# halide/Halide

Measured on AMD Instinct MI355X. Metric: megapixels/sec local_laplacian 8-level fp32 4K, higher is better.
Workload: dtype f32; 1 GPU; apps/local_laplacian J=8 levels=8 alpha=1/7 beta=1, u16 RGB planar 3840x2160; distinct_frames_per_gpu=8, lut_cached=True, streams_per_gpu=4, frame_scheduling=4 frame-queue streams, boundary=C ABI local_laplacian(halide_buffer_t*,int32,float,float,halide_buffer_t*), rccl_ranks=1, parallelism=frames sharded over 1 GPU(s), no data-path collective

## Files before the change

### halide_amd/csrc/local_laplacian.hip

```cpp
#include "hlmi_device_math.h"
#include "hlmi_internal.h"

#include <atomic>
#include <mutex>
#include <optional>
#include <stdlib.h>
#include <string.h>
#include <type_traits>

using namespace hlmi;

namespace {

constexpr int J = 8;
constexpr int MAX_K = 32;
constexpr int STRIP = 126;
constexpr int KCH = 8;
constexpr int D0_THREADS = 256;

struct Level {
    int lox, loy;
    int w, h;
    int ws;
    size_t ps;
// ... 2007 lines not shown
        stage1(y + 2, f0, s0, g0);
        __builtin_amdgcn_sched_barrier(0);
        stage2(y + 1, s1, g1);
        __builtin_amdgcn_sched_barrier(0);
    }
    LL_PROBE_T(pt3);
    LL_PROBE_ADD(8, pt1 - pt0); LL_PROBE_ADD(9, pt2 - pt1); LL_PROBE_ADD(10, 1);
    LL_PROBE_ADD(11, pt3 - pt2); LL_PROBE_ADD(12, pt3 - pt0);
}

struct Up0HArgs {
    Up0Args u;
    const float *outl0;
    int l0_ws;
    int fuse2;
    const float *g3, *out3;
    int lox3, loy3, ws3;
    size_t ps3;
};
constexpr int U0H_PF = 4;
constexpr int U0H_T2 = 68;
template<bool NT, bool EM1, int CH = 2>
__global__ __launch_bounds__(256) void ll_up0h(Up0HArgs ph, Geometry gm) {
    const Up0Args &p = ph.u;
    LL_RESIDENCY(1);
    extern __shared__ float s_out1[];
    int bx, by;
    {
        const int b = (int)blockIdx.y * (int)gridDim.x + (int)blockIdx.x, nb8 = (int)(gridDim.x * gridDim.y) >> 3;
        const int lb = b < (nb8 << 3) ? (b & 7) * nb8 + (b >> 3) : b;
        by = lb / (int)gridDim.x, bx = lb - by * (int)gridDim.x;
    }
    const int X0 = p.ox0 + bx * 256;
    const int Yw0 = p.oy0 + by * (2 * p.RU);
    const int Yw1 = min(Yw0 + 2 * p.RU, p.oy0 + p.oh) - 1;
    const int cx0 = (X0 >> 1) - 1, cy0 = dev::fdiv2(Yw0 - 1);
    const int th = dev::fdiv2(Yw1 + 1) - cy0 + 1;
    float *const s_out2 = s_out1 + U0_TS * (p.RU + 2);
    const int cx1 = min(cx0 + U0_TW - 1, p.rx1_1);
    const int c2x0 = dev::fdiv2(cx0 - 1), c2y0 = dev::fdiv2(cy0 - 1);
    struct Taps32 {
        uint32_t b, a;
    };
    auto mul24 = [](uint32_t a, uint32_t b) { return (uint32_t)__umul24(a, b); };
    auto tap_bytes = [&](uint32_t row0, int y0, int lox, int ws, int X, int Y) {
        Taps32 t;
        t.b = (row0 + mul24((uint32_t)(dev::fdiv2(Y - 1) - y0), (uint32_t)ws) + (uint32_t)(dev::fdiv2(X - 1) - lox)) << 2;
        t.a = t.b + ((uint32_t)ws << 2);
        return t;
    };
    auto taps_at = [](const float *base, uint32_t plane_bytes, const Taps32 &t) {
        const F2U lo = ld_su<F2U>(base, plane_bytes + t.b), hi = ld_su<F2U>(base, plane_bytes + t.a);
        UpTaps r;
        r.bb = lo.x, r.ba = lo.y, r.ab = hi.x, r.aa = hi.y;
        return r;
    };
    const uint32_t ps1b = (uint32_t)p.ps1 * 4u, ps2b = (uint32_t)p.ps2 * 4u, ps3b = (uint32_t)ph.ps3 * 4u;
    if (ph.fuse2) {
        const int n2x = dev::fdiv2(cx1 + 1) - c2x0 + 1, n2y = dev::fdiv2(cy0 + th) - c2y0 + 1, n2 = n2x * n2y;
        const uint32_t m2 = (4194304u + (uint32_t)n2x - 1u) / (uint32_t)n2x;
        const int c3y0 = dev::fdiv2(c2y0 - 1);
        const uint32_t row2 = (uint32_t)((c2y0 - p.loy2) * p.ws2), row3 = (uint32_t)((c3y0 - ph.loy3) * ph.ws3);
        for (int e0 = threadIdx.x; e0 < n2; e0 += 256 * CH) {
            int X2[CH], Y2[CH];
            uint32_t ti[CH];
            bool ok[CH];
            uint32_t ob[CH];
            Taps32 t3[CH];
            float inG[CH], lf[CH], ga[CH], gb[CH];
            UpTaps o3[CH], t0[CH], t1[CH];
#pragma unroll
            for (int i = 0; i < CH; i++) {
                const int e = e0 + 256 * i;
                const uint32_t ec = (uint32_t)min(e, n2 - 1), ty = mul24(ec, m2) >> 22, tx = ec - mul24(ty, (uint32_t)n2x);
                ok[i] = e < n2, ti[i] = mul24(ty, U0H_T2) + tx;
                X2[i] = c2x0 + (int)tx, Y2[i] = c2y0 + (int)ty;
                ob[i] = (row2 + mul24(ty, (uint32_t)p.ws2) + (uint32_t)(X2[i] - p.lox2)) << 2;
                inG[i] = ld_su<float>(p.g2, (uint32_t)gm.K * ps2b + ob[i]);
                t3[i] = tap_bytes(row3, c3y0, ph.lox3, ph.ws3, X2[i], Y2[i]);
                o3[i] = taps_at(ph.out3, 0u, t3[i]);
            }
            __builtin_amdgcn_sched_barrier(0);
#pragma unroll
            for (int i = 0; i < CH; i++) {
                const float level = inG[i] * gm.Km1;
                const int li = dev::clampi((int)level, 0, gm.K - 2);
                lf[i] = level - (float)li;
                ga[i] = ld_su<float>(p.g2, (uint32_t)li * ps2b + ob[i]), gb[i] = ld_su<float>(p.g2, (uint32_t)(li + 1) * ps2b + ob[i]);
                t0[i] = taps_at(ph.g3, (uint32_t)li * ps3b, t3[i]);
                t1[i] = taps_at(ph.g3, (uint32_t)(li + 1) * ps3b, t3[i]);
            }
            __builtin_amdgcn_sched_barrier(0);
#pragma unroll
            for (int i = 0; i < CH; i++) {
                const float l0 = ga[i] - up_from(t0[i], X2[i], Y2[i]), l1 = gb[i] - up_from(t1[i], X2[i], Y2[i]);
                const float outL = dev::mad2(1.0f - lf[i], l0, lf[i], l1);
                if (ok[i]) s_out2[ti[i]] = up_from(o3[i], X2[i], Y2[i]) + outL;
            }
        }
        __syncthreads();
    }
    {
        const int n1 = U0_TW * th;
        constexpr uint32_t M1 = (4194304u + U0_TW - 1) / U0_TW;
        const uint32_t row1 = (uint32_t)((cy0 - p.loy1) * p.ws1), row2 = (uint32_t)((c2y0 - p.loy2) * p.ws2);
        if constexpr (EM1) {
            for (int e0 = threadIdx.x; e0 < n1; e0 += 256 * CH) {
                int cx[CH], cy[CH];
                uint32_t ti[CH];
                bool ok[CH];
                float outL[CH];
#pragma unroll
                for (int i = 0; i < CH; i++) {
                    const int e = e0 + 256 * i;
                    const uint32_t ec = (uint32_t)min(e, n1 - 1), ty = mul24(ec, M1) >> 22, tx = ec - mul24(ty, U0_TW);
                    ok[i] = e < n1 && cx0 + (int)tx <= p.rx1_1, ti[i] = mul24(ty, U0_TS) + tx;
                    cx[i] = min(cx0 + (int)tx, p.rx1_1), cy[i] = cy0 + (int)ty;
                    outL[i] = ld_su<float>(p.g1, (row1 + mul24(ty, (uint32_t)p.ws1) + (uint32_t)(cx[i] - p.lox1)) << 2);
                }
#pragma unroll
                for (int i = 0; i < CH; i++) {
                    const float *q = s_out2 + mul24((uint32_t)(dev::fdiv2(cy[i] - 1) - c2y0), U0H_T2) + (uint32_t)(dev::fdiv2(cx[i] - 1) - c2x0);
                    UpTaps t;
                    t.bb = q[0], t.ba = q[1], t.ab = q[U0H_T2], t.aa = q[U0H_T2 + 1];
                    if (ok[i]) s_out1[ti[i]] = up_from(t, cx[i], cy[i]) + outL[i];
                }
            }
        } else {
            for (int e0 = threadIdx.x; e0 < n1; e0 += 256 * CH) {
                int cx[CH], cy[CH];
                uint32_t ti[CH];
                bool ok[CH];
                Taps32 t2[CH];
                float inG[CH], lf[CH], ga[CH], gb[CH];
                UpTaps o2[CH], t0[CH], t1[CH];
#pragma unroll
                for (int i = 0; i < CH; i++) {
                    const int e = e0 + 256 * i;
                    const uint32_t ec = (uint32_t)min(e, n1 - 1), ty = mul24(ec, M1) >> 22, tx = ec - mul24(ty, U0_TW);
                    ok[i] = e < n1 && cx0 + (int)tx <= p.rx1_1, ti[i] = mul24(ty, U0_TS) + tx;
                    cx[i] = min(cx0 + (int)tx, p.rx1_1), cy[i] = cy0 + (int)ty;
                    const uint32_t ob = (row1 + mul24(ty, (uint32_t)p.ws1) + (uint32_t)(cx[i] - p.lox1)) << 2;
                    inG[i] = ld_su<float>(p.g1, (uint32_t)gm.K * ps1b + ob), ga[i] = ld_su<float>(p.g1, ob), gb[i] = ld_su<float>(p.g1, ps1b + ob);
                    t2[i] = tap_bytes(row2, c2y0, p.lox2, p.ws2, cx[i], cy[i]);
                    if (!ph.fuse2) o2[i] = taps_at(p.out2, 0u, t2[i]);
                }
                __builtin_amdgcn_sched_barrier(0);
#pragma unroll
                for (int i = 0; i < CH; i++) {
                    const float level = inG[i] * gm.Km1;
                    const int li = dev::clampi((int)level, 0, gm.K - 2);
                    lf[i] = level - (float)li;
                    t0[i] = taps_at(p.g2, (uint32_t)li * ps2b, t2[i]);
                    t1[i] = taps_at(p.g2, (uint32_t)(li + 1) * ps2b, t2[i]);
                }
                __builtin_amdgcn_sched_barrier(0);
#pragma unroll
                for (int i = 0; i < CH; i++) {
                    const float l0 = ga[i] - up_from(t0[i], cx[i], cy[i]), l1 = gb[i] - up_from(t1[i], cx[i], cy[i]);
                    const float outL = dev::mad2(1.0f - lf[i], l0, lf[i], l1);
                    float up2;
                    if (ph.fuse2) {
                        const float *q = s_out2 + mul24((uint32_t)(dev::fdiv2(cy[i] - 1) - c2y0), U0H_T2) + (uint32_t)(dev::fdiv2(cx[i] - 1) - c2x0);
                        UpTaps t;
                        t.bb = q[0], t.ba = q[1], t.ab = q[U0H_T2], t.aa = q[U0H_T2 + 1];
                        up2 = up_from(t, cx[i], cy[i]);
                    } else {
                        up2 = up_from(o2[i], cx[i], cy[i]);
                    }
                    if (ok[i]) s_out1[ti[i]] = up2 + outL;
                }
            }
        }
    }
    __syncthreads();
    const int wave = __builtin_amdgcn_readfirstlane(threadIdx.x >> 6), lane = threadIdx.x & 63;
    const int x = bx * 256 + (wave & 1) * 128 + 2 * lane;
    const int y0 = by * (2 * p.RU) + (wave >> 1) * p.RU;
    if (y0 >= p.oh || x >= p.ow) return;
    const int y1 = min(y0 + p.RU, p.oh);
    const int X = p.ox0 + x;
    uint32_t inb = (uint32_t)(X - gm.ix0) * 2u, outb = (uint32_t)x * 2u, l0b = (uint32_t)(X - gm.ix0) * 4u;
    auto hl0 = [](float rm, float r0) {
        return dev::CANON_FMA ? __builtin_fmaf(r0, 0.75f, rm * 0.25f) : __builtin_fmaf(rm, 0.25f, r0 * 0.75f);
    };
    auto hl1 = [](float r0, float rp) { return __builtin_fmaf(rp, 0.25f, r0 * 0.75f); };
    auto vl = [](float uq, float ut, float wq, float wt) {
        return dev::CANON_FMA ? __builtin_fmaf(uq, wq, ut * wt) : __builtin_fmaf(uq, 0.25f, ut * 0.75f);
    };
    struct Frame {
        ushort2 c0, c1, c2;
        float2 l0;
    };
    auto fresh = [](uint32_t &v) {
        asm volatile("" : "+v"(v));
        return v;
    };
    auto load_frame = [&](int y, Frame &f) {
        const int yc = min(y, y1 - 1);
        const uint16_t *irow = p.in + (long)(p.oy0 + yc - gm.iy0) * p.in_sy;
        const uint32_t ib = fresh(inb);
        f.c0 = ld_frame2<NT>(irow + p.gco[0], ib), f.c1 = ld_frame2<NT>(irow + p.gco[1], ib), f.c2 = ld_frame2<NT>(irow + p.gco[2], ib);
        {
            const f2 *const lp = reinterpret_cast<const f2 *>(reinterpret_cast<const char *>(ph.outl0 + (size_t)yc * ph.l0_ws) + fresh(l0b));
            const f2 v = NT ? __builtin_nontemporal_load(lp) : *lp;
            f.l0 = make_float2(v.x, v.y);
        }
    };
    auto finish = [&](int y, const Frame &f) {
        const int Y = p.oy0 + min(y, y1 - 1);
        const int ya = dev::fdiv2(Y + 1), yb = dev::fdiv2(Y - 1);
        const bool yodd = dev::fmod2(Y) != 0;
        const int yq = (dev::CANON_FMA || yodd) ? ya : yb, yt = (dev::CANON_FMA || yodd) ? yb : ya;
        const float wq = yodd ? 0.25f : 0.75f, wt = yodd ? 0.75f : 0.25f;
        const float *oa = s_out1 + (yq - cy0) * U0_TS + (wave & 1) * 64 + lane;
        const float *ob = s_out1 + (yt - cy0) * U0_TS + (wave & 1) * 64 + lane;
        const float ax = oa[0], ay = oa[1], az = oa[2], bx = ob[0], by = ob[1], bz = ob[2];
        const float uo[2] = {vl(hl0(ax, ay), hl0(bx, by), wq, wt), vl(hl1(ay, az), hl1(by, bz), wq, wt)};
        const float outL[2] = {f.l0.x, f.l0.y};
        const uint16_t ch[3][2] = {{f.c0.x, f.c0.y}, {f.c1.x, f.c1.y}, {f.c2.x, f.c2.y}};
        uint16_t res[3][2];
#pragma unroll
        for (int i = 0; i < 2; i++) {
            const float gray = gray_from(ch[0][i], ch[1][i], ch[2][i]);
            const float og = (uo[i] + outL[i]) + 0.01f;
            const float gr = gray + 0.01f;
            const float n[3] = {(float)ch[0][i] * og, (float)ch[1][i] * og, (float)ch[2][i] * og};
            float q[3];
            div3_by(n, gr, q);
#pragma unroll
            for (int c = 0; c < 3; c++) res[c][i] = (uint16_t)__builtin_amdgcn_fmed3f(q[c], 0.0f, 65535.0f);
        }
        if (y < y1) {
            uint16_t *orow = p.out + (long)y * p.out_sy;
#pragma unroll
            for (int c = 0; c < 3; c++) st_frame2<NT>(reinterpret_cast<char *>(orow + (long)c * p.out_sc) + fresh(outb), res[c][0], res[c][1]);
        }
    };
    Frame f[U0H_PF];
#pragma unroll
    for (int i = 0; i < U0H_PF; i++) load_frame(y0 + i, f[i]);
    for (int y = y0; y < y1; y += U0H_PF) {
#pragma unroll
        for (int i = 0; i < U0H_PF; i++) {
            const Frame cur = f[i];
            load_frame(y + U0H_PF + i, f[i]);
            finish(y + i, cur);
        }
    }
}

const ArgTable ll_table("local_laplacian", {
    in_buf("input", T_U16, 3, {0, 1536, 0, 2560, 0, 3}),
    scalar_i32("levels").estimate(8),
    scalar_f32("alpha").estimate(1),
    scalar_f32("beta").estimate(1),
    out_buf("output", T_U16, 3, {0, 1536, 0, 2560, 0, 3}),
});

struct LlSwitches {
    std::optional<int> fuse_from, upchain_from, ru, units0, no_vec, emit, nt, fuse_up2, d01_exch, d01_pad_lds, no_lut_cache, emit1, chain_fit;
};
LlSwitches ll_switches() {
    const auto get = env_int;
    LlSwitches s;
    s.fuse_from = get("HLMI_LL_FUSE_FROM"), s.upchain_from = get("HLMI_LL_UPCHAIN_FROM");
    s.ru = get("HLMI_LL_RU"), s.units0 = get("HLMI_LL_UNITS0"), s.no_vec = get("HLMI_LL_NO_VEC");
    s.emit = get("HLMI_LL_EMIT"), s.nt = get("HLMI_LL_NT"), s.fuse_up2 = get("HLMI_LL_FUSE_UP2");
    s.d01_exch = get("HLMI_LL_D01_EXCH"), s.d01_pad_lds = get("HLMI_LL_D01_PAD_LDS"), s.no_lut_cache = get("HLMI_LL_NO_LUT_CACHE");
    s.emit1 = get("HLMI_LL_EMIT1"), s.chain_fit = get("HLMI_LL_CHAIN_FIT");
    return s;
}

int dev_clamp_ru(int ru) { return ru < 1 ? 1 : (ru > 300 ? 300 : ru); }

struct PairGeom {
    int S2;
    int Pbase;
    int nsx;
};
struct LlPlan {
    Geometry gm;
    Level lv[J];
    size_t off_g[J], off_out[J], off_l0, ws_floats;
    Up0Args u0;
    int nlut;
    int S, SU;
    int up_low;
    bool lut_cache;
    bool lut_lds;
    bool vec_frame;
    bool vec_in;
    bool b1;
    bool fast, fuse1, fuse2, emit, nt;
    bool emit1;
    bool d01;
    bool strip2;
    bool chain_fit;
    struct { PairGeom pg; bool exch; int nsy, nunits; size_t lds; } d0;
    struct { PairGeom pg; int nsy, nunits; } s2;
    int units_strip;
    size_t up0_lds;
};

struct LlBuffers {
    float *lut, *outl0;
    float *g[J], *outg[J];
};

PairGeom pair_geom(const Level &d, const Level &e, int fewer = 0) {
    PairGeom g;
    g.S2 = ((d.odd || e.odd) ? 62 : 61) - fewer;
    const int lim = e.odd ? 2 * e.lox - 1 : 2 * e.lox - 2;
    g.Pbase = min(d.lox, lim);
    const int hi1 = d.lox + d.w - 1, hi2 = e.lox + e.w - 1;
    const int x2_first = e.odd ? (g.Pbase + 1) / 2 + 0 : g.Pbase / 2 + 1;
    g.nsx = max((hi2 - x2_first + g.S2) / g.S2, (hi1 - g.Pbase + 2 * g.S2) / (2 * g.S2));
    return g;
// ... 67 lines not shown
        const int v = sw.upchain_from.value_or(S == 4 ? 3 : 0);
        return (v >= 1 && v <= J - 2) ? v : S;
    }();
    const bool partitioned = stream_cus < device_cus;
    bool vec_frame = (din % 4 == 0) && (dout % 4 == 0) && in_sy % 2 == 0 && out_sy % 2 == 0 && out_sc % 2 == 0 &&
                     ((p.ox0 - gm.ix0) % 2 == 0) && !sw.no_vec.value_or(0);
    for (int ch = 0; ch < 3; ch++) vec_frame = vec_frame && p.gco[ch] % 2 == 0 && p.cco[ch] % 2 == 0;
    pl.vec_frame = vec_frame;
    const bool vec_in = pl.vec_in = (din % 8 == 0) && in_sy % 4 == 0 && p.gco[0] % 4 == 0 && p.gco[1] % 4 == 0 && p.gco[2] % 4 == 0 &&
                                    iw % 4 == 0 && !sw.no_vec.value_or(0);
    const bool fast = pl.fast = vec_frame && same && nc == 3 && (ow & 1) == 0 && (p.ox0 & 1) == 0 &&
                                (double)(levels + 1) * (4.0 * (double)lv[1].ps) < 4.0e9;
    const bool fuse1 = pl.fuse1 = fast && SU >= 2;
    const bool d01 = pl.d01 = levels == KCH && lut_lds && vec_in;
    const bool emit = pl.emit = d01 && fast && fuse1 && lv[1].ws < (1 << 24) && sw.emit.value_or(1);
    int RU = dev_clamp_ru(sw.ru.value_or(emit ? (partitioned ? 32 : 8) : fuse1 ? (partitioned ? 32 : 16) : 8));
    pl.nt = sw.nt.value_or(partitioned ? 1 : 0) != 0;
    pl.fuse2 = emit && SU >= 3 && SU < J && sw.fuse_up2.value_or(1);
    pl.up_low = fuse1 ? (pl.fuse2 ? 3 : 2) : 1;
    constexpr bool kEmit1Default = true;
    constexpr size_t kCuLds = 160 * 1024, kLdsGranule = 1280;
    constexpr int WPB = D0_THREADS / 64;
    auto lds_alloc = [](size_t bytes) { return (bytes + kLdsGranule - 1) / kLdsGranule * kLdsGranule; };
    auto up0h_lds = [](int ru) { return sizeof(float) * ((size_t)U0_TS * (ru + 2) + (size_t)U0H_T2 * (ru / 2 + 4)); };
    const size_t d01_lds_exch = sizeof(float) * ((nlut + 1) & ~1) + sizeof(float2) * D01_STATE * (2 * WPB - 1);
    pl.emit1 = false;
    {
        const int e1 = sw.emit1.value_or(-1);
        if (pl.fuse2 && (e1 > 0 || (e1 < 0 && partitioned && kEmit1Default))) {
            const size_t d0 = lds_alloc(d01_lds_exch + d01_em1_lds_bytes());
            auto fits = [&](int ru) { return d0 + 3 * lds_alloc(up0h_lds(ru)) <= kCuLds; };
            int ru = RU;
            if (partitioned && !sw.ru) {
                ru &= ~3;
                while (ru > 8 && !fits(ru)) ru -= 4;
            }
            pl.emit1 = e1 > 0 || fits(ru);
            if (pl.emit1) RU = ru;
        }
    }
    p.RU = RU;
    pl.strip2 = d01 && S == 4;

    pl.off_l0 = ws_floats;
    if (emit) ws_floats += ((size_t)iw * (size_t)oh + 63) & ~(size_t)63;
    pl.ws_floats = ws_floats;

    if (!d01) {
        const Level &d = lv[1];
        const int target = sw.units0.value_or(8 * device_cus);
        pl.d0.nsy = max(1, min(max(target / d.nsx, (d.h + 63) / 64), max(1, d.h / 2)));
        pl.d0.nunits = d.nsx * pl.d0.nsy;
        pl.d0.lds = (lut_lds ? sizeof(float) * ((nlut + 1) & ~1) : 0) + sizeof(float2) * D0_THREADS * (KCH + 1);
    } else {
        const Level &e = lv[2];
        const PairGeom pg = pl.d0.pg = pair_geom(lv[1], e, pl.emit1 ? (e.odd ? 1 : 2) : 0);
        const int target2 = sw.units0.value_or(emit && partitioned ? 10 * stream_cus : 8 * device_cus);
        bool exch = sw.d01_exch.value_or(1) != 0;
        int nwy = 0;
        auto ceil_div = [](int x, int y) { return (x + y - 1) / y; };
        if (exch) {
            const int nwy_max = max(1, target2 / (WPB * pg.nsx));
            const int n = max(2, (ceil_div(e.h, nwy_max) + 1 + 3) / 4);
// ... 2 lines not shown
        }
        pl.d0.exch = exch;
        if (exch) {
            pl.d0.nsy = nwy;
            pl.d0.nunits = pg.nsx * nwy * WPB;
        } else {
            pl.d0.nsy = max(1, min(max(target2 / pg.nsx, (e.h + 31) / 32), e.h));
            pl.d0.nunits = pg.nsx * pl.d0.nsy;
        }
        size_t sh2 = sizeof(float) * ((nlut + 1) & ~1) + sizeof(float2) * D01_STATE * (WPB + (exch ? WPB - 1 : 0));
        if (pl.emit1) sh2 += d01_em1_lds_bytes();
        const int pad = sw.d01_pad_lds.value_or(emit && partitioned ? -1 : 0);
        constexpr size_t kHalfCuLds = 160 * 1024 / 2;
        if (pad < 0) sh2 = max(sh2, kHalfCuLds + 2048);
        else sh2 += (size_t)pad;
        pl.d0.lds = sh2;
    }
    if (pl.strip2) {
        pl.s2.pg = pair_geom(lv[3], lv[4]);
        pl.s2.nsy = (lv[4].h + S2_RPU - 1) / S2_RPU;
        pl.s2.nunits = (levels + 1) * pl.s2.pg.nsx * pl.s2.nsy;
    }
    pl.units_strip = 16 * device_cus;
    pl.up0_lds = emit   ? sizeof(float) * ((size_t)U0_TS * (RU + 2) + (size_t)U0H_T2 * (RU / 2 + 4))
                 : fast ? lut_sh + (fuse1 ? ((lut_lds && (nlut & 1)) ? 4 : 0) + sizeof(float) * U0_TS * (RU + 2) : 0)
                        : lut_sh;
    {
        const int cf = (double)(levels + 1) * (4.0 * (double)lv[1].ps) < 4.0e9 ? sw.chain_fit.value_or(-1) : 0;
        const size_t taken = lds_alloc(pl.d0.lds) + 3 * lds_alloc(pl.up0_lds);
        const size_t need = max(S < J - 1 ? lds_alloc(dm_lds_bytes(J - 1 - S)) : (size_t)0, SU < J - 1 ? lds_alloc(um_lds_bytes(J - 1 - SU)) : (size_t)0);
        pl.chain_fit = cf > 0 || (cf < 0 && pl.emit1 && partitioned && taken + need <= kCuLds);
    }
}

struct LlLastCall {
    LlPlan pl;
    LlBuffers b;
    hipStream_t stream;
    bool out1_pending;
    bool out2_pending;
};
thread_local LlLastCall t_dbg = {};

StripArgs strip_args(const LlPlan &pl, const LlBuffers &b, int j) {
    const Level &sl = pl.lv[j], &d = pl.lv[j + 1];
    const int cols = d.nsx * (pl.gm.K + 1);
    StripArgs a;
// ... 179 lines not shown
        HLMI_LAUNCH(uc, nm, st, ll_up<false>, dim3((ua.rw + 255) / 256, ua.rh), dim3(256), 0, ua);
    }
    return 0;
}

int ll_stage_up0(void *uc, const LlPlan &pl, const LlBuffers &b, hipStream_t st) {
    const Geometry &gm = pl.gm;
    const Level *lv = pl.lv;
    const Level &c = lv[1];
    Up0Args p = pl.u0;
    const int ow = p.ow, oh = p.oh, nc = p.nc;
    p.lut_g = b.lut, p.g1 = b.g[1], p.out1 = b.outg[1];
    p.lox1 = c.lox, p.loy1 = c.loy, p.ws1 = c.ws, p.ps1 = c.ps;
    p.g2 = b.g[2], p.out2 = b.outg[2], p.lox2 = lv[2].lox, p.loy2 = lv[2].loy, p.ws2 = lv[2].ws, p.ps2 = lv[2].ps;
    p.rx1_1 = c.rx1, p.rx0_1 = c.rx0, p.ry0_1 = c.ry0, p.ry1_1 = c.ry1;
    dim3 grid((ow + 255) / 256, (oh + 2 * p.RU - 1) / (2 * p.RU)), block(256);
    const double n1 = (double)(c.rx1 - c.rx0 + 1) * (c.ry1 - c.ry0 + 1), n2 = (double)(lv[2].rx1 - lv[2].rx0 + 1) * (lv[2].ry1 - lv[2].ry0 + 1);
    if (pl.emit) {
        timing_note_bytes(2.0 * (3 + nc) * ow * oh + 4.0 * ow * oh + 4.0 * (pl.emit1 ? 1.0 : 3.0) * n1 + 4.0 * 3.0 * n2);
        Up0HArgs ph;
        ph.u = p, ph.outl0 = b.outl0, ph.l0_ws = gm.ix1 - gm.ix0 + 1;
        ph.fuse2 = pl.fuse2 ? 1 : 0;
        ph.g3 = b.g[3], ph.out3 = b.outg[3], ph.lox3 = lv[3].lox, ph.loy3 = lv[3].loy, ph.ws3 = lv[3].ws, ph.ps3 = lv[3].ps;
        return with_flags([&](auto NT, auto E1) -> int {
            HLMI_LAUNCH(uc, "ll_up0", st, (ll_up0h<NT.value, E1.value>), grid, block, pl.up0_lds, ph, gm);
            return 0;
        }, pl.nt, pl.emit1);
    }
    timing_note_bytes(2.0 * (3 + nc) * ow * oh + 4.0 * 3.0 * n1 + (pl.fuse1 ? 4.0 * 3.0 * n2 : 0.0));
    if (pl.fast) {
        return with_flags([&](auto L, auto B, auto F) -> int {
            HLMI_LAUNCH(uc, "ll_up0", st, (ll_up0f<L.value, B.value, F.value>), grid, block, pl.up0_lds, p, gm);
            return 0;
        }, pl.lut_lds, pl.b1, pl.fuse1);
    }
    return with_flags([&](auto V, auto L) -> int {
        HLMI_LAUNCH(uc, "ll_up0", st, (ll_up0<V.value, L.value>), grid, block, pl.up0_lds, p, gm);
        return 0;
    }, pl.vec_frame, pl.lut_lds);
}

}

extern "C" int local_laplacian(halide_buffer_t *input, int32_t levels, float alpha, float beta, halide_buffer_t *output) {
    void *uc = nullptr;
    const LlSwitches sw = ll_switches();
// ... 169 lines not shown
```

Measured before the change: 125,400 Mpx/s.

## Stream level-1 rows per wave in up0h instead of staging a full LDS tile

Adds an ll_up0r variant of the fused level-0 upsample kernel. It computes level-1 coarse rows on the fly, one row per wave, using DPP lane shifts plus a small per-wave edge buffer for horizontal neighbours, instead of first materialising the whole level-1 tile in LDS. This shrinks per-block LDS, which lets the planner use a taller RU (64) while still fitting three blocks per CU. The cost is a more complex kernel with wave-level synchronisation, and horizontal-edge values get recomputed. The variant is enabled by default on partitioned emit1 plans.

```diff
diff --git a/halide_amd/csrc/local_laplacian.hip b/halide_amd/csrc/local_laplacian.hip
--- a/halide_amd/csrc/local_laplacian.hip
+++ b/halide_amd/csrc/local_laplacian.hip
@@ -2053,232 +2053,14 @@
 constexpr int U0H_T2 = 68;
 template<bool NT, bool EM1, int CH = 2>
 __global__ __launch_bounds__(256) void ll_up0h(Up0HArgs ph, Geometry gm) {
-    const Up0Args &p = ph.u;
-    LL_RESIDENCY(1);
-    extern __shared__ float s_out1[];
-    int bx, by;
-    {
-        const int b = (int)blockIdx.y * (int)gridDim.x + (int)blockIdx.x, nb8 = (int)(gridDim.x * gridDim.y) >> 3;
-        const int lb = b < (nb8 << 3) ? (b & 7) * nb8 + (b >> 3) : b;
-        by = lb / (int)gridDim.x, bx = lb - by * (int)gridDim.x;
-    }
-    const int X0 = p.ox0 + bx * 256;
-    const int Yw0 = p.oy0 + by * (2 * p.RU);
-    const int Yw1 = min(Yw0 + 2 * p.RU, p.oy0 + p.oh) - 1;
-    const int cx0 = (X0 >> 1) - 1, cy0 = dev::fdiv2(Yw0 - 1);
-    const int th = dev::fdiv2(Yw1 + 1) - cy0 + 1;
-    float *const s_out2 = s_out1 + U0_TS * (p.RU + 2);
-    const int cx1 = min(cx0 + U0_TW - 1, p.rx1_1);
-    const int c2x0 = dev::fdiv2(cx0 - 1), c2y0 = dev::fdiv2(cy0 - 1);
-    struct Taps32 {
-        uint32_t b, a;
-    };
-    auto mul24 = [](uint32_t a, uint32_t b) { return (uint32_t)__umul24(a, b); };
-    auto tap_bytes = [&](uint32_t row0, int y0, int lox, int ws, int X, int Y) {
-        Taps32 t;
-        t.b = (row0 + mul24((uint32_t)(dev::fdiv2(Y - 1) - y0), (uint32_t)ws) + (uint32_t)(dev::fdiv2(X - 1) - lox)) << 2;
-        t.a = t.b + ((uint32_t)ws << 2);
-        return t;
-    };
-    auto taps_at = [](const float *base, uint32_t plane_bytes, const Taps32 &t) {
-        const F2U lo = ld_su<F2U>(base, plane_bytes + t.b), hi = ld_su<F2U>(base, plane_bytes + t.a);
-        UpTaps r;
-        r.bb = lo.x, r.ba = lo.y, r.ab = hi.x, r.aa = hi.y;
-        return r;
-    };
-    const uint32_t ps1b = (uint32_t)p.ps1 * 4u, ps2b = (uint32_t)p.ps2 * 4u, ps3b = (uint32_t)ph.ps3 * 4u;
-    if (ph.fuse2) {
-        const int n2x = dev::fdiv2(cx1 + 1) - c2x0 + 1, n2y = dev::fdiv2(cy0 + th) - c2y0 + 1, n2 = n2x * n2y;
-        const uint32_t m2 = (4194304u + (uint32_t)n2x - 1u) / (uint32_t)n2x;
-        const int c3y0 = dev::fdiv2(c2y0 - 1);
-        const uint32_t row2 = (uint32_t)((c2y0 - p.loy2) * p.ws2), row3 = (uint32_t)((c3y0 - ph.loy3) * ph.ws3);
-        for (int e0 = threadIdx.x; e0 < n2; e0 += 256 * CH) {
-            int X2[CH], Y2[CH];
-            uint32_t ti[CH];
-            bool ok[CH];
-            uint32_t ob[CH];
-            Taps32 t3[CH];
-            float inG[CH], lf[CH], ga[CH], gb[CH];
-            UpTaps o3[CH], t0[CH], t1[CH];
-#pragma unroll
-            for (int i = 0; i < CH; i++) {
-                const int e = e0 + 256 * i;
-                const uint32_t ec = (uint32_t)min(e, n2 - 1), ty = mul24(ec, m2) >> 22, tx = ec - mul24(ty, (uint32_t)n2x);
-                ok[i] = e < n2, ti[i] = mul24(ty, U0H_T2) + tx;
-                X2[i] = c2x0 + (int)tx, Y2[i] = c2y0 + (int)ty;
-                ob[i] = (row2 + mul24(ty, (uint32_t)p.ws2) + (uint32_t)(X2[i] - p.lox2)) << 2;
-                inG[i] = ld_su<float>(p.g2, (uint32_t)gm.K * ps2b + ob[i]);
-                t3[i] = tap_bytes(row3, c3y0, ph.lox3, ph.ws3, X2[i], Y2[i]);
-                o3[i] = taps_at(ph.out3, 0u, t3[i]);
-            }
-            __builtin_amdgcn_sched_barrier(0);
-#pragma unroll
-            for (int i = 0; i < CH; i++) {
-                const float level = inG[i] * gm.Km1;
-                const int li = dev::clampi((int)level, 0, gm.K - 2);
-                lf[i] = level - (float)li;
-                ga[i] = ld_su<float>(p.g2, (uint32_t)li * ps2b + ob[i]), gb[i] = ld_su<float>(p.g2, (uint32_t)(li + 1) * ps2b + ob[i]);
-                t0[i] = taps_at(ph.g3, (uint32_t)li * ps3b, t3[i]);
-                t1[i] = taps_at(ph.g3, (uint32_t)(li + 1) * ps3b, t3[i]);
-            }
-            __builtin_amdgcn_sched_barrier(0);
-#pragma unroll
-            for (int i = 0; i < CH; i++) {
-                const float l0 = ga[i] - up_from(t0[i], X2[i], Y2[i]), l1 = gb[i] - up_from(t1[i], X2[i], Y2[i]);
-                const float outL = dev::mad2(1.0f - lf[i], l0, lf[i], l1);
-                if (ok[i]) s_out2[ti[i]] = up_from(o3[i], X2[i], Y2[i]) + outL;
-            }
-        }
-        __syncthreads();
-    }
-    {
-        const int n1 = U0_TW * th;
-        constexpr uint32_t M1 = (4194304u + U0_TW - 1) / U0_TW;
-        const uint32_t row1 = (uint32_t)((cy0 - p.loy1) * p.ws1), row2 = (uint32_t)((c2y0 - p.loy2) * p.ws2);
-        if constexpr (EM1) {
-            for (int e0 = threadIdx.x; e0 < n1; e0 += 256 * CH) {
-                int cx[CH], cy[CH];
-                uint32_t ti[CH];
-                bool ok[CH];
-                float outL[CH];
-#pragma unroll
-                for (int i = 0; i < CH; i++) {
-                    const int e = e0 + 256 * i;
-                    const uint32_t ec = (uint32_t)min(e, n1 - 1), ty = mul24(ec, M1) >> 22, tx = ec - mul24(ty, U0_TW);
-                    ok[i] = e < n1 && cx0 + (int)tx <= p.rx1_1, ti[i] = mul24(ty, U0_TS) + tx;
-                    cx[i] = min(cx0 + (int)tx, p.rx1_1), cy[i] = cy0 + (int)ty;
-                    outL[i] = ld_su<float>(p.g1, (row1 + mul24(ty, (uint32_t)p.ws1) + (uint32_t)(cx[i] - p.lox1)) << 2);
-                }
-#pragma unroll
-                for (int i = 0; i < CH; i++) {
-                    const float *q = s_out2 + mul24((uint32_t)(dev::fdiv2(cy[i] - 1) - c2y0), U0H_T2) + (uint32_t)(dev::fdiv2(cx[i] - 1) - c2x0);
-                    UpTaps t;
-                    t.bb = q[0], t.ba = q[1], t.ab = q[U0H_T2], t.aa = q[U0H_T2 + 1];
-                    if (ok[i]) s_out1[ti[i]] = up_from(t, cx[i], cy[i]) + outL[i];
-                }
-            }
-        } else {
-            for (int e0 = threadIdx.x; e0 < n1; e0 += 256 * CH) {
-                int cx[CH], cy[CH];
-                uint32_t ti[CH];
-                bool ok[CH];
-                Taps32 t2[CH];
-                float inG[CH], lf[CH], ga[CH], gb[CH];
-                UpTaps o2[CH], t0[CH], t1[CH];
-#pragma unroll
-                for (int i = 0; i < CH; i++) {
-                    const int e = e0 + 256 * i;
-                    const uint32_t ec = (uint32_t)min(e, n1 - 1), ty = mul24(ec, M1) >> 22, tx = ec - mul24(ty, U0_TW);
-                    ok[i] = e < n1 && cx0 + (int)tx <= p.rx1_1, ti[i] = mul24(ty, U0_TS) + tx;
-                    cx[i] = min(cx0 + (int)tx, p.rx1_1), cy[i] = cy0 + (int)ty;
-                    const uint32_t ob = (row1 + mul24(ty, (uint32_t)p.ws1) + (uint32_t)(cx[i] - p.lox1)) << 2;
-                    inG[i] = ld_su<float>(p.g1, (uint32_t)gm.K * ps1b + ob), ga[i] = ld_su<float>(p.g1, ob), gb[i] = ld_su<float>(p.g1, ps1b + ob);
-                    t2[i] = tap_bytes(row2, c2y0, p.lox2, p.ws2, cx[i], cy[i]);
-                    if (!ph.fuse2) o2[i] = taps_at(p.out2, 0u, t2[i]);
-                }
-                __builtin_amdgcn_sched_barrier(0);
-#pragma unroll
-                for (int i = 0; i < CH; i++) {
-                    const float level = inG[i] * gm.Km1;
-                    const int li = dev::clampi((int)level, 0, gm.K - 2);
-                    lf[i] = level - (float)li;
-                    t0[i] = taps_at(p.g2, (uint32_t)li * ps2b, t2[i]);
-                    t1[i] = taps_at(p.g2, (uint32_t)(li + 1) * ps2b, t2[i]);
-                }
-                __builtin_amdgcn_sched_barrier(0);
-#pragma unroll
-                for (int i = 0; i < CH; i++) {
-                    const float l0 = ga[i] - up_from(t0[i], cx[i], cy[i]), l1 = gb[i] - up_from(t1[i], cx[i], cy[i]);
-                    const float outL = dev::mad2(1.0f - lf[i], l0, lf[i], l1);
-                    float up2;
-                    if (ph.fuse2) {
-                        const float *q = s_out2 + mul24((uint32_t)(dev::fdiv2(cy[i] - 1) - c2y0), U0H_T2) + (uint32_t)(dev::fdiv2(cx[i] - 1) - c2x0);
-                        UpTaps t;
-                        t.bb = q[0], t.ba = q[1], t.ab = q[U0H_T2], t.aa = q[U0H_T2 + 1];
-                        up2 = up_from(t, cx[i], cy[i]);
-                    } else {
-                        up2 = up_from(o2[i], cx[i], cy[i]);
-                    }
-                    if (ok[i]) s_out1[ti[i]] = up2 + outL;
-                }
-            }
-        }
-    }
-    __syncthreads();
-    const int wave = __builtin_amdgcn_readfirstlane(threadIdx.x >> 6), lane = threadIdx.x & 63;
-    const int x = bx * 256 + (wave & 1) * 128 + 2 * lane;
-    const int y0 = by * (2 * p.RU) + (wave >> 1) * p.RU;
-    if (y0 >= p.oh || x >= p.ow) return;
-    const int y1 = min(y0 + p.RU, p.oh);
-    const int X = p.ox0 + x;
-    uint32_t inb = (uint32_t)(X - gm.ix0) * 2u, outb = (uint32_t)x * 2u, l0b = (uint32_t)(X - gm.ix0) * 4u;
-    auto hl0 = [](float rm, float r0) {
-        return dev::CANON_FMA ? __builtin_fmaf(r0, 0.75f, rm * 0.25f) : __builtin_fmaf(rm, 0.25f, r0 * 0.75f);
-    };
-    auto hl1 = [](float r0, float rp) { return __builtin_fmaf(rp, 0.25f, r0 * 0.75f); };
-    auto vl = [](float uq, float ut, float wq, float wt) {
-        return dev::CANON_FMA ? __builtin_fmaf(uq, wq, ut * wt) : __builtin_fmaf(uq, 0.25f, ut * 0.75f);
-    };
-    struct Frame {
-        ushort2 c0, c1, c2;
-        float2 l0;
-    };
-    auto fresh = [](uint32_t &v) {
-        asm volatile("" : "+v"(v));
-        return v;
-    };
-    auto load_frame = [&](int y, Frame &f) {
-        const int yc = min(y, y1 - 1);
-        const uint16_t *irow = p.in + (long)(p.oy0 + yc - gm.iy0) * p.in_sy;
-        const uint32_t ib = fresh(inb);
-        f.c0 = ld_frame2<NT>(irow + p.gco[0], ib), f.c1 = ld_frame2<NT>(irow + p.gco[1], ib), f.c2 = ld_frame2<NT>(irow + p.gco[2], ib);
-        {
-            const f2 *const lp = reinterpret_cast<const f2 *>(reinterpret_cast<const char *>(ph.outl0 + (size_t)yc * ph.l0_ws) + fresh(l0b));
-            const f2 v = NT ? __builtin_nontemporal_load(lp) : *lp;
-            f.l0 = make_float2(v.x, v.y);
-        }
-    };
-    auto finish = [&](int y, const Frame &f) {
-        const int Y = p.oy0 + min(y, y1 - 1);
-        const int ya = dev::fdiv2(Y + 1), yb = dev::fdiv2(Y - 1);
-        const bool yodd = dev::fmod2(Y) != 0;
-        const int yq = (dev::CANON_FMA || yodd) ? ya : yb, yt = (dev::CANON_FMA || yodd) ? yb : ya;
-        const float wq = yodd ? 0.25f : 0.75f, wt = yodd ? 0.75f : 0.25f;
-        const float *oa = s_out1 + (yq - cy0) * U0_TS + (wave & 1) * 64 + lane;
-        const float *ob = s_out1 + (yt - cy0) * U0_TS + (wave & 1) * 64 + lane;
-        const float ax = oa[0], ay = oa[1], az = oa[2], bx = ob[0], by = ob[1], bz = ob[2];
-        const float uo[2] = {vl(hl0(ax, ay), hl0(bx, by), wq, wt), vl(hl1(ay, az), hl1(by, bz), wq, wt)};
-        const float outL[2] = {f.l0.x, f.l0.y};
-        const uint16_t ch[3][2] = {{f.c0.x, f.c0.y}, {f.c1.x, f.c1.y}, {f.c2.x, f.c2.y}};
-        uint16_t res[3][2];
-#pragma unroll
-        for (int i = 0; i < 2; i++) {
-            const float gray = gray_from(ch[0][i], ch[1][i], ch[2][i]);
-            const float og = (uo[i] + outL[i]) + 0.01f;
-            const float gr = gray + 0.01f;
-            const float n[3] = {(float)ch[0][i] * og, (float)ch[1][i] * og, (float)ch[2][i] * og};
-            float q[3];
-            div3_by(n, gr, q);
-#pragma unroll
-            for (int c = 0; c < 3; c++) res[c][i] = (uint16_t)__builtin_amdgcn_fmed3f(q[c], 0.0f, 65535.0f);
-        }
-        if (y < y1) {
-            uint16_t *orow = p.out + (long)y * p.out_sy;
-#pragma unroll
-            for (int c = 0; c < 3; c++) st_frame2<NT>(reinterpret_cast<char *>(orow + (long)c * p.out_sc) + fresh(outb), res[c][0], res[c][1]);
-        }
-    };
-    Frame f[U0H_PF];
-#pragma unroll
-    for (int i = 0; i < U0H_PF; i++) load_frame(y0 + i, f[i]);
-    for (int y = y0; y < y1; y += U0H_PF) {
-#pragma unroll
-        for (int i = 0; i < U0H_PF; i++) {
-            const Frame cur = f[i];
-            load_frame(y + U0H_PF + i, f[i]);
-            finish(y + i, cur);
-        }
-    }
+    constexpr bool ROWS1 = false;
+#include "local_laplacian_up0h_body.h"
+}
+template<bool NT>
+__global__ __launch_bounds__(256) void ll_up0r(Up0HArgs ph, Geometry gm) {
+    constexpr bool EM1 = true, ROWS1 = true;
+    constexpr int CH = 2;
+#include "local_laplacian_up0h_body.h"
 }
 
 const ArgTable ll_table("local_laplacian", {
@@ -2290,7 +2072,7 @@
 });
 
 struct LlSwitches {
-    std::optional<int> fuse_from, upchain_from, ru, units0, no_vec, emit, nt, fuse_up2, d01_exch, d01_pad_lds, no_lut_cache, emit1, chain_fit;
+    std::optional<int> fuse_from, upchain_from, ru, units0, no_vec, emit, nt, fuse_up2, d01_exch, d01_pad_lds, no_lut_cache, emit1, chain_fit, up1_rows;
 };
 LlSwitches ll_switches() {
     const auto get = env_int;
@@ -2299,7 +2081,7 @@
     s.ru = get("HLMI_LL_RU"), s.units0 = get("HLMI_LL_UNITS0"), s.no_vec = get("HLMI_LL_NO_VEC");
     s.emit = get("HLMI_LL_EMIT"), s.nt = get("HLMI_LL_NT"), s.fuse_up2 = get("HLMI_LL_FUSE_UP2");
     s.d01_exch = get("HLMI_LL_D01_EXCH"), s.d01_pad_lds = get("HLMI_LL_D01_PAD_LDS"), s.no_lut_cache = get("HLMI_LL_NO_LUT_CACHE");
-    s.emit1 = get("HLMI_LL_EMIT1"), s.chain_fit = get("HLMI_LL_CHAIN_FIT");
+    s.emit1 = get("HLMI_LL_EMIT1"), s.chain_fit = get("HLMI_LL_CHAIN_FIT"), s.up1_rows = get("HLMI_LL_UP1_ROWS");
     return s;
 }
 
@@ -2325,6 +2107,7 @@
     bool b1;
     bool fast, fuse1, fuse2, emit, nt;
     bool emit1;
+    bool up1_rows;
     bool d01;
     bool strip2;
     bool chain_fit;
@@ -2438,16 +2221,22 @@
     constexpr size_t kCuLds = 160 * 1024, kLdsGranule = 1280;
     constexpr int WPB = D0_THREADS / 64;
     auto lds_alloc = [](size_t bytes) { return (bytes + kLdsGranule - 1) / kLdsGranule * kLdsGranule; };
-    auto up0h_lds = [](int ru) { return sizeof(float) * ((size_t)U0_TS * (ru + 2) + (size_t)U0H_T2 * (ru / 2 + 4)); };
+    auto up0h_lds = [](int ru, bool rows1) {
+        return sizeof(float) * ((rows1 ? (size_t)(256 / 64) * 2 * (ru / 2 + 2) : (size_t)U0_TS * (ru + 2)) + (size_t)U0H_T2 * (ru / 2 + 4));
+    };
     const size_t d01_lds_exch = sizeof(float) * ((nlut + 1) & ~1) + sizeof(float2) * D01_STATE * (2 * WPB - 1);
+    constexpr int kRows1Ru = 64;
     pl.emit1 = false;
+    bool rows1 = false;
     {
-        const int e1 = sw.emit1.value_or(-1);
+        const int e1 = sw.emit1.value_or(-1), u1 = sw.up1_rows.value_or(-1);
         if (pl.fuse2 && (e1 > 0 || (e1 < 0 && partitioned && kEmit1Default))) {
+            rows1 = u1 > 0 || (u1 < 0 && partitioned);
             const size_t d0 = lds_alloc(d01_lds_exch + d01_em1_lds_bytes());
-            auto fits = [&](int ru) { return d0 + 3 * lds_alloc(up0h_lds(ru)) <= kCuLds; };
+            auto fits = [&](int ru) { return d0 + 3 * lds_alloc(up0h_lds(ru, rows1)) <= kCuLds; };
             int ru = RU;
             if (partitioned && !sw.ru) {
+                if (rows1) ru = kRows1Ru;
                 ru &= ~3;
                 while (ru > 8 && !fits(ru)) ru -= 4;
             }
@@ -2455,6 +2244,7 @@
             if (pl.emit1) RU = ru;
         }
     }
+    pl.up1_rows = pl.emit1 && rows1;
     p.RU = RU;
     pl.strip2 = d01 && S == 4;
 
@@ -2503,7 +2293,7 @@
         pl.s2.nunits = (levels + 1) * pl.s2.pg.nsx * pl.s2.nsy;
     }
     pl.units_strip = 16 * device_cus;
-    pl.up0_lds = emit   ? sizeof(float) * ((size_t)U0_TS * (RU + 2) + (size_t)U0H_T2 * (RU / 2 + 4))
+    pl.up0_lds = emit   ? up0h_lds(RU, pl.up1_rows)
                  : fast ? lut_sh + (fuse1 ? ((lut_lds && (nlut & 1)) ? 4 : 0) + sizeof(float) * U0_TS * (RU + 2) : 0)
                         : lut_sh;
     {
@@ -2729,6 +2519,12 @@
         ph.u = p, ph.outl0 = b.outl0, ph.l0_ws = gm.ix1 - gm.ix0 + 1;
         ph.fuse2 = pl.fuse2 ? 1 : 0;
         ph.g3 = b.g[3], ph.out3 = b.outg[3], ph.lox3 = lv[3].lox, ph.loy3 = lv[3].loy, ph.ws3 = lv[3].ws, ph.ps3 = lv[3].ps;
+        if (pl.up1_rows) {
+            return with_flags([&](auto NT) -> int {
+                HLMI_LAUNCH(uc, "ll_up0r", st, (ll_up0r<NT.value>), grid, block, pl.up0_lds, ph, gm);
+                return 0;
+            }, pl.nt);
+        }
         return with_flags([&](auto NT, auto E1) -> int {
             HLMI_LAUNCH(uc, "ll_up0", st, (ll_up0h<NT.value, E1.value>), grid, block, pl.up0_lds, ph, gm);
             return 0;
diff --git a/halide_amd/csrc/local_laplacian_up0h_body.h b/halide_amd/csrc/local_laplacian_up0h_body.h
--- /dev/null
+++ b/halide_amd/csrc/local_laplacian_up0h_body.h
@@ -0,0 +1,326 @@
+    static_assert(EM1 || !ROWS1, "ROWS1 adds the stored outLPyramid[1] plane");
+    const Up0Args &p = ph.u;
+    LL_RESIDENCY(1);
+    extern __shared__ float s_out1[];
+    int bx, by;
+    {
+        const int b = (int)blockIdx.y * (int)gridDim.x + (int)blockIdx.x, nb8 = (int)(gridDim.x * gridDim.y) >> 3;
+        const int lb = b < (nb8 << 3) ? (b & 7) * nb8 + (b >> 3) : b;
+        by = lb / (int)gridDim.x, bx = lb - by * (int)gridDim.x;
+    }
+    const int X0 = p.ox0 + bx * 256;
+    const int Yw0 = p.oy0 + by * (2 * p.RU);
+    const int Yw1 = min(Yw0 + 2 * p.RU, p.oy0 + p.oh) - 1;
+    const int cx0 = (X0 >> 1) - 1, cy0 = dev::fdiv2(Yw0 - 1);
+    const int th = dev::fdiv2(Yw1 + 1) - cy0 + 1;
+    float *const s_out2 = s_out1 + (ROWS1 ? 0 : U0_TS * (p.RU + 2));
+    const int cx1 = min(cx0 + U0_TW - 1, p.rx1_1);
+    const int c2x0 = dev::fdiv2(cx0 - 1), c2y0 = dev::fdiv2(cy0 - 1);
+    struct Taps32 {
+        uint32_t b, a;
+    };
+    auto mul24 = [](uint32_t a, uint32_t b) { return (uint32_t)__umul24(a, b); };
+    auto tap_bytes = [&](uint32_t row0, int y0, int lox, int ws, int X, int Y) {
+        Taps32 t;
+        t.b = (row0 + mul24((uint32_t)(dev::fdiv2(Y - 1) - y0), (uint32_t)ws) + (uint32_t)(dev::fdiv2(X - 1) - lox)) << 2;
+        t.a = t.b + ((uint32_t)ws << 2);
+        return t;
+    };
+    auto taps_at = [](const float *base, uint32_t plane_bytes, const Taps32 &t) {
+        const F2U lo = ld_su<F2U>(base, plane_bytes + t.b), hi = ld_su<F2U>(base, plane_bytes + t.a);
+        UpTaps r;
+        r.bb = lo.x, r.ba = lo.y, r.ab = hi.x, r.aa = hi.y;
+        return r;
+    };
+    const uint32_t ps1b = (uint32_t)p.ps1 * 4u, ps2b = (uint32_t)p.ps2 * 4u, ps3b = (uint32_t)ph.ps3 * 4u;
+    if (ph.fuse2) {
+        const int n2x = dev::fdiv2(cx1 + 1) - c2x0 + 1, n2y = dev::fdiv2(cy0 + th) - c2y0 + 1, n2 = n2x * n2y;
+        const uint32_t m2 = (4194304u + (uint32_t)n2x - 1u) / (uint32_t)n2x;
+        const int c3y0 = dev::fdiv2(c2y0 - 1);
+        const uint32_t row2 = (uint32_t)((c2y0 - p.loy2) * p.ws2), row3 = (uint32_t)((c3y0 - ph.loy3) * ph.ws3);
+        for (int e0 = threadIdx.x; e0 < n2; e0 += 256 * CH) {
+            int X2[CH], Y2[CH];
+            uint32_t ti[CH];
+            bool ok[CH];
+            uint32_t ob[CH];
+            Taps32 t3[CH];
+            float inG[CH], lf[CH], ga[CH], gb[CH];
+            UpTaps o3[CH], t0[CH], t1[CH];
+#pragma unroll
+            for (int i = 0; i < CH; i++) {
+                const int e = e0 + 256 * i;
+                const uint32_t ec = (uint32_t)min(e, n2 - 1), ty = mul24(ec, m2) >> 22, tx = ec - mul24(ty, (uint32_t)n2x);
+                ok[i] = e < n2, ti[i] = mul24(ty, U0H_T2) + tx;
+                X2[i] = c2x0 + (int)tx, Y2[i] = c2y0 + (int)ty;
+                ob[i] = (row2 + mul24(ty, (uint32_t)p.ws2) + (uint32_t)(X2[i] - p.lox2)) << 2;
+                inG[i] = ld_su<float>(p.g2, (uint32_t)gm.K * ps2b + ob[i]);
+                t3[i] = tap_bytes(row3, c3y0, ph.lox3, ph.ws3, X2[i], Y2[i]);
+                o3[i] = taps_at(ph.out3, 0u, t3[i]);
+            }
+            __builtin_amdgcn_sched_barrier(0);
+#pragma unroll
+            for (int i = 0; i < CH; i++) {
+                const float level = inG[i] * gm.Km1;
+                const int li = dev::clampi((int)level, 0, gm.K - 2);
+                lf[i] = level - (float)li;
+                ga[i] = ld_su<float>(p.g2, (uint32_t)li * ps2b + ob[i]), gb[i] = ld_su<float>(p.g2, (uint32_t)(li + 1) * ps2b + ob[i]);
+                t0[i] = taps_at(ph.g3, (uint32_t)li * ps3b, t3[i]);
+                t1[i] = taps_at(ph.g3, (uint32_t)(li + 1) * ps3b, t3[i]);
+            }
+            __builtin_amdgcn_sched_barrier(0);
+#pragma unroll
+            for (int i = 0; i < CH; i++) {
+                const float l0 = ga[i] - up_from(t0[i], X2[i], Y2[i]), l1 = gb[i] - up_from(t1[i], X2[i], Y2[i]);
+                const float outL = dev::mad2(1.0f - lf[i], l0, lf[i], l1);
+                if (ok[i]) s_out2[ti[i]] = up_from(o3[i], X2[i], Y2[i]) + outL;
+            }
+        }
+        __syncthreads();
+    }
+    if constexpr (!ROWS1) {
+        const int n1 = U0_TW * th;
+        constexpr uint32_t M1 = (4194304u + U0_TW - 1) / U0_TW;
+        const uint32_t row1 = (uint32_t)((cy0 - p.loy1) * p.ws1), row2 = (uint32_t)((c2y0 - p.loy2) * p.ws2);
+        if constexpr (EM1) {
+            for (int e0 = threadIdx.x; e0 < n1; e0 += 256 * CH) {
+                int cx[CH], cy[CH];
+                uint32_t ti[CH];
+                bool ok[CH];
+                float outL[CH];
+#pragma unroll
+                for (int i = 0; i < CH; i++) {
+                    const int e = e0 + 256 * i;
+                    const uint32_t ec = (uint32_t)min(e, n1 - 1), ty = mul24(ec, M1) >> 22, tx = ec - mul24(ty, U0_TW);
+                    ok[i] = e < n1 && cx0 + (int)tx <= p.rx1_1, ti[i] = mul24(ty, U0_TS) + tx;
+                    cx[i] = min(cx0 + (int)tx, p.rx1_1), cy[i] = cy0 + (int)ty;
+                    outL[i] = ld_su<float>(p.g1, (row1 + mul24(ty, (uint32_t)p.ws1) + (uint32_t)(cx[i] - p.lox1)) << 2);
+                }
+#pragma unroll
+                for (int i = 0; i < CH; i++) {
+                    const float *q = s_out2 + mul24((uint32_t)(dev::fdiv2(cy[i] - 1) - c2y0), U0H_T2) + (uint32_t)(dev::fdiv2(cx[i] - 1) - c2x0);
+                    UpTaps t;
+                    t.bb = q[0], t.ba = q[1], t.ab = q[U0H_T2], t.aa = q[U0H_T2 + 1];
+                    if (ok[i]) s_out1[ti[i]] = up_from(t, cx[i], cy[i]) + outL[i];
+                }
+            }
+        } else {
+            for (int e0 = threadIdx.x; e0 < n1; e0 += 256 * CH) {
+                int cx[CH], cy[CH];
+                uint32_t ti[CH];
+                bool ok[CH];
+                Taps32 t2[CH];
+                float inG[CH], lf[CH], ga[CH], gb[CH];
+                UpTaps o2[CH], t0[CH], t1[CH];
+#pragma unroll
+                for (int i = 0; i < CH; i++) {
+                    const int e = e0 + 256 * i;
+                    const uint32_t ec = (uint32_t)min(e, n1 - 1), ty = mul24(ec, M1) >> 22, tx = ec - mul24(ty, U0_TW);
+                    ok[i] = e < n1 && cx0 + (int)tx <= p.rx1_1, ti[i] = mul24(ty, U0_TS) + tx;
+                    cx[i] = min(cx0 + (int)tx, p.rx1_1), cy[i] = cy0 + (int)ty;
+                    const uint32_t ob = (row1 + mul24(ty, (uint32_t)p.ws1) + (uint32_t)(cx[i] - p.lox1)) << 2;
+                    inG[i] = ld_su<float>(p.g1, (uint32_t)gm.K * ps1b + ob), ga[i] = ld_su<float>(p.g1, ob), gb[i] = ld_su<float>(p.g1, ps1b + ob);
+                    t2[i] = tap_bytes(row2, c2y0, p.lox2, p.ws2, cx[i], cy[i]);
+                    if (!ph.fuse2) o2[i] = taps_at(p.out2, 0u, t2[i]);
+                }
+                __builtin_amdgcn_sched_barrier(0);
+#pragma unroll
+                for (int i = 0; i < CH; i++) {
+                    const float level = inG[i] * gm.Km1;
+                    const int li = dev::clampi((int)level, 0, gm.K - 2);
+                    lf[i] = level - (float)li;
+                    t0[i] = taps_at(p.g2, (uint32_t)li * ps2b, t2[i]);
+                    t1[i] = taps_at(p.g2, (uint32_t)(li + 1) * ps2b, t2[i]);
+                }
+                __builtin_amdgcn_sched_barrier(0);
+#pragma unroll
+                for (int i = 0; i < CH; i++) {
+                    const float l0 = ga[i] - up_from(t0[i], cx[i], cy[i]), l1 = gb[i] - up_from(t1[i], cx[i], cy[i]);
+                    const float outL = dev::mad2(1.0f - lf[i], l0, lf[i], l1);
+                    float up2;
+                    if (ph.fuse2) {
+                        const float *q = s_out2 + mul24((uint32_t)(dev::fdiv2(cy[i] - 1) - c2y0), U0H_T2) + (uint32_t)(dev::fdiv2(cx[i] - 1) - c2x0);
+                        UpTaps t;
+                        t.bb = q[0], t.ba = q[1], t.ab = q[U0H_T2], t.aa = q[U0H_T2 + 1];
+                        up2 = up_from(t, cx[i], cy[i]);
+                    } else {
+                        up2 = up_from(o2[i], cx[i], cy[i]);
+                    }
+                    if (ok[i]) s_out1[ti[i]] = up2 + outL;
+                }
+            }
+        }
+    }
+    if constexpr (!ROWS1) __syncthreads();
+    const int wave = __builtin_amdgcn_readfirstlane(threadIdx.x >> 6), lane = threadIdx.x & 63;
+    const int x = bx * 256 + (wave & 1) * 128 + 2 * lane;
+    const int y0 = by * (2 * p.RU) + (wave >> 1) * p.RU;
+    if (y0 >= p.oh || (ROWS1 ? x - 2 * lane : x) >= p.ow) return;
+    const bool live = x < p.ow;
+    const int y1 = min(y0 + p.RU, p.oh);
+    const int X = p.ox0 + (ROWS1 ? min(x, p.ow - 2) : x);
+    uint32_t inb = (uint32_t)(X - gm.ix0) * 2u, outb = (uint32_t)x * 2u, l0b = (uint32_t)(X - gm.ix0) * 4u;
+    auto hl0 = [](float rm, float r0) {
+        return dev::CANON_FMA ? __builtin_fmaf(r0, 0.75f, rm * 0.25f) : __builtin_fmaf(rm, 0.25f, r0 * 0.75f);
+    };
+    auto hl1 = [](float r0, float rp) { return __builtin_fmaf(rp, 0.25f, r0 * 0.75f); };
+    auto vl = [](float uq, float ut, float wq, float wt) {
+        return dev::CANON_FMA ? __builtin_fmaf(uq, wq, ut * wt) : __builtin_fmaf(uq, 0.25f, ut * 0.75f);
+    };
+    struct Frame {
+        ushort2 c0, c1, c2;
+        float2 l0;
+    };
+    auto fresh = [](uint32_t &v) {
+        asm volatile("" : "+v"(v));
+        return v;
+    };
+    auto load_frame = [&](int y, Frame &f) {
+        const int yc = min(y, y1 - 1);
+        const uint16_t *irow = p.in + (long)(p.oy0 + yc - gm.iy0) * p.in_sy;
+        const uint32_t ib = fresh(inb);
+        f.c0 = ld_frame2<NT>(irow + p.gco[0], ib), f.c1 = ld_frame2<NT>(irow + p.gco[1], ib), f.c2 = ld_frame2<NT>(irow + p.gco[2], ib);
+        {
+            const f2 *const lp = reinterpret_cast<const f2 *>(reinterpret_cast<const char *>(ph.outl0 + (size_t)yc * ph.l0_ws) + (ROWS1 ? 2u * fresh(inb) : fresh(l0b)));
+            const f2 v = NT ? __builtin_nontemporal_load(lp) : *lp;
+            f.l0 = make_float2(v.x, v.y);
+        }
+    };
+    if constexpr (!ROWS1) {
+        auto finish = [&](int y, const Frame &f) {
+            const int Y = p.oy0 + min(y, y1 - 1);
+            const int ya = dev::fdiv2(Y + 1), yb = dev::fdiv2(Y - 1);
+            const bool yodd = dev::fmod2(Y) != 0;
+            const int yq = (dev::CANON_FMA || yodd) ? ya : yb, yt = (dev::CANON_FMA || yodd) ? yb : ya;
+            const float wq = yodd ? 0.25f : 0.75f, wt = yodd ? 0.75f : 0.25f;
+            const float *oa = s_out1 + (yq - cy0) * U0_TS + (wave & 1) * 64 + lane;
+            const float *ob = s_out1 + (yt - cy0) * U0_TS + (wave & 1) * 64 + lane;
+            const float ax = oa[0], ay = oa[1], az = oa[2], bx = ob[0], by = ob[1], bz = ob[2];
+            const float uo[2] = {vl(hl0(ax, ay), hl0(bx, by), wq, wt), vl(hl1(ay, az), hl1(by, bz), wq, wt)};
+            const float outL[2] = {f.l0.x, f.l0.y};
+            const uint16_t ch[3][2] = {{f.c0.x, f.c0.y}, {f.c1.x, f.c1.y}, {f.c2.x, f.c2.y}};
+            uint16_t res[3][2];
+#pragma unroll
+            for (int i = 0; i < 2; i++) {
+                const float gray = gray_from(ch[0][i], ch[1][i], ch[2][i]);
+                const float og = (uo[i] + outL[i]) + 0.01f;
+                const float gr = gray + 0.01f;
+                const float n[3] = {(float)ch[0][i] * og, (float)ch[1][i] * og, (float)ch[2][i] * og};
+                float q[3];
+                div3_by(n, gr, q);
+#pragma unroll
+                for (int c = 0; c < 3; c++) res[c][i] = (uint16_t)__builtin_amdgcn_fmed3f(q[c], 0.0f, 65535.0f);
+            }
+            if (y < y1) {
+                uint16_t *orow = p.out + (long)y * p.out_sy;
+#pragma unroll
+                for (int c = 0; c < 3; c++) st_frame2<NT>(reinterpret_cast<char *>(orow + (long)c * p.out_sc) + fresh(outb), res[c][0], res[c][1]);
+            }
+        };
+        Frame f[U0H_PF];
+#pragma unroll
+        for (int i = 0; i < U0H_PF; i++) load_frame(y0 + i, f[i]);
+        for (int y = y0; y < y1; y += U0H_PF) {
+#pragma unroll
+            for (int i = 0; i < U0H_PF; i++) {
+                const Frame cur = f[i];
+                load_frame(y + U0H_PF + i, f[i]);
+                finish(y + i, cur);
+            }
+        }
+    } else {
+        auto recolour = [&](int y, const Frame &f, const float (&uo)[2]) {
+            const float outL[2] = {f.l0.x, f.l0.y};
+            const uint16_t ch[3][2] = {{f.c0.x, f.c0.y}, {f.c1.x, f.c1.y}, {f.c2.x, f.c2.y}};
+            uint16_t res[3][2];
+#pragma unroll
+            for (int i = 0; i < 2; i++) {
+                const float gray = gray_from(ch[0][i], ch[1][i], ch[2][i]);
+                const float og = (uo[i] + outL[i]) + 0.01f;
+                const float gr = gray + 0.01f;
+                const float n[3] = {(float)ch[0][i] * og, (float)ch[1][i] * og, (float)ch[2][i] * og};
+                float q[3];
+                div3_by(n, gr, q);
+#pragma unroll
+                for (int c = 0; c < 3; c++) res[c][i] = (uint16_t)__builtin_amdgcn_fmed3f(q[c], 0.0f, 65535.0f);
+            }
+            if (y < y1 && live) {
+                uint16_t *orow = p.out + (long)y * p.out_sy;
+#pragma unroll
+                for (int c = 0; c < 3; c++) st_frame2<NT>(reinterpret_cast<char *>(orow + (long)c * p.out_sc) + fresh(outb), res[c][0], res[c][1]);
+            }
+        };
+        const int c0 = (X0 >> 1) + (wave & 1) * 64;
+        const int cc = min(c0 + lane, p.rx1_1);
+        const int m0 = dev::fdiv2(p.oy0 + y0 - 1), mlast = dev::fdiv2(p.oy0 + y1);
+        uint32_t c1b = (uint32_t)(cc - p.lox1) * 4u, ln = (uint32_t)lane;
+        const float *const qc = s_out2 + (dev::fdiv2(cc - 1) - c2x0);
+        auto g1_at = [&](const float *q, float outL, int cx, int m) {
+            UpTaps t;
+            t.bb = q[0], t.ba = q[1], t.ab = q[U0H_T2], t.aa = q[U0H_T2 + 1];
+            return up_from(t, cx, m) + outL;
+        };
+        float *const s_edge = s_out2 + U0H_T2 * (p.RU / 2 + 4) + wave * (2 * (p.RU / 2 + 2));
+        {
+            const uint32_t row1 = (uint32_t)((m0 - p.loy1) * p.ws1);
+            for (int e = lane; e < 2 * (mlast - m0 + 1); e += 64) {
+                const int m = m0 + (e >> 1), cx = (e & 1) ? min(c0 + 64, p.rx1_1) : c0 - 1;
+                const float outL = ld_su<float>(p.g1, (row1 + mul24((uint32_t)(e >> 1), (uint32_t)p.ws1) + (uint32_t)(cx - p.lox1)) << 2);
+                s_edge[e] = g1_at(s_out2 + mul24((uint32_t)(dev::fdiv2(m - 1) - c2y0), U0H_T2) + (dev::fdiv2(cx - 1) - c2x0), outL, cx, m);
+            }
+            __builtin_amdgcn_fence(__ATOMIC_RELEASE, "wavefront");
+            __builtin_amdgcn_wave_barrier();
+            __builtin_amdgcn_fence(__ATOMIC_ACQUIRE, "wavefront");
+        }
+        auto load_row1 = [&](int m, float &l) {
+            l = ld_su<float>(p.g1 + (long)(min(m, mlast) - p.loy1) * p.ws1, fresh(c1b));
+        };
+        auto coarse_row = [&](int m, float l, float (&h)[2]) {
+            const int mc = min(m, mlast);
+            const float g = g1_at(qc + mul24((uint32_t)(dev::fdiv2(mc - 1) - c2y0), U0H_T2), l, cc, mc);
+            const uint32_t lu = fresh(ln);
+            const float e = s_edge[2 * (mc - m0) + (int)(lu >> 5)];
+            const float gm1 = __builtin_bit_cast(float, __builtin_amdgcn_update_dpp(__builtin_bit_cast(int, e), __builtin_bit_cast(int, g), 0x138, 0xf, 0xf, false));
+            const float gp1 = __builtin_bit_cast(float, __builtin_amdgcn_update_dpp(__builtin_bit_cast(int, e), __builtin_bit_cast(int, g), 0x130, 0xf, 0xf, false));
+            h[0] = hl0(gm1, g), h[1] = hl1(g, gp1);
+            __builtin_amdgcn_sched_barrier(0);
+        };
+        auto rows = [&](auto P) {
+            constexpr bool ODD = decltype(P)::value;
+            const int Yf = p.oy0 + y0;
+            float lo[2] = {0.0f, 0.0f}, hi[2];
+            Frame f[U0H_PF];
+            float r1[U0H_PF / 2], ra, rb = 0.0f;
+            load_row1(dev::fdiv2(Yf - 1), ra);
+            if (!ODD) load_row1(dev::fdiv2(Yf + 1), rb);
+#pragma unroll
+            for (int i = 0; i < U0H_PF; i++) {
+                load_frame(y0 + i, f[i]);
+                if (ODD != ((i & 1) != 0)) load_row1(dev::fdiv2(Yf + i + 1), r1[i >> 1]);
+            }
+            coarse_row(dev::fdiv2(Yf - 1), ra, hi);
+            if (!ODD) {
+                lo[0] = hi[0], lo[1] = hi[1];
+                coarse_row(dev::fdiv2(Yf + 1), rb, hi);
+            }
+            for (int y = y0; y < y1; y += U0H_PF) {
+#pragma unroll
+                for (int i = 0; i < U0H_PF; i++) {
+                    const bool yodd = ODD != ((i & 1) != 0);
+                    if (yodd) {
+                        lo[0] = hi[0], lo[1] = hi[1];
+                        coarse_row(dev::fdiv2(p.oy0 + y + i + 1), r1[i >> 1], hi);
+                    }
+                    const bool qhi = dev::CANON_FMA || yodd;
+                    const float wq = yodd ? 0.25f : 0.75f, wt = yodd ? 0.75f : 0.25f;
+                    const float uo[2] = {vl(qhi ? hi[0] : lo[0], qhi ? lo[0] : hi[0], wq, wt), vl(qhi ? hi[1] : lo[1], qhi ? lo[1] : hi[1], wq, wt)};
+                    recolour(y + i, f[i], uo);
+                    __builtin_amdgcn_sched_barrier(0);
+                    load_frame(y + U0H_PF + i, f[i]);
+                    if (yodd) load_row1(dev::fdiv2(p.oy0 + y + U0H_PF + i + 1), r1[i >> 1]);
+                    __builtin_amdgcn_sched_barrier(0);
+                }
+            }
+        };
+        if (dev::fmod2(p.oy0 + y0) != 0) rows(std::true_type{});
+        else rows(std::false_type{});
+    }
```

After: 129,300 Mpx/s (median of 6 runs). 3.1% higher.
